# highfem/tqdne

Measured on AMD Instinct MI355X. Metric: waveforms/sec (train step + 18-step EDM sample), 3ch x 4096, higher is better.
Workload: dtype f32 (contractions on MFMA with fp32 accumulate: bf16x3, and fp16 + block-scaled-fp6 corrections on the 128/256-channel forward convs; sampler state f64)

## Files before the change

### tqdne_amd/csrc/backward.hip

```cpp
#include <cstdlib>
#include "common.hpp"
#include "../../include/tqdne_hip.h"

using namespace tq;

namespace {

typedef short s16x4 __attribute__((ext_vector_type(4)));

__device__ __forceinline__ f32x4 wg_mma(const bf16x8& ah, const bf16x8& al, const bf16x8& bh, const bf16x8& bl, f32x4 c) {
#if defined(TQ_WG_ABL_HIHI)
    return mfma_bf16(ah, bh, c);
#elif defined(TQ_WG_ABL_HALF)
    c = mfma_bf16(ah, bl, c);
    return mfma_bf16(ah, bh, c);
#else
    return mfma_x3(ah, al, bh, bl, c);
#endif
}

__device__ __forceinline__ uint2 lds_tr_read(const unsigned char* p) {
    s16x4 v = __builtin_amdgcn_ds_read_tr16_b64_v4i16((__attribute__((address_space(3))) s16x4*)(p));
    union { s16x4 s; uint2 u; } c;
    c.s = v;
// ... 187 lines not shown
                if (p.flags & TQ_CONV_SILU) {
#pragma unroll
                    for (int j = 0; j < 4; ++j) v[j] = silu_f(v[j]);
                }
                if (p.flags & TQ_CONV_DROPOUT) {
                    const uint32_t e0 = (uint32_t)pos * (uint32_t)Cin + (uint32_t)(cb + 4 * m);
                    const DropKey dkey = drop_key(p.drop_seed, p.drop_site, (uint32_t)b);
#pragma unroll
                    for (int j = 0; j < 4; ++j)
                        v[j] = (drop_hash(dkey, e0 + j) >= p.drop_thresh) ? v[j] * p.drop_scale : 0.f;
                }
            }
            bf16x4 h, l;
#pragma unroll
            for (int j = 0; j < 4; ++j) { __bf16 hh, ll; split_bf16(v[j], hh, ll); h[j] = hh; l[j] = ll; }
            const int off = i * WG_X_STRIDE + (W8 ? ((m * 8) ^ wg_x_swz128(i)) : (NCI == 1 ? ((m * 8) ^ wg_x_swz(i)) : (NCI == 4 ? ((m * 8) ^ wg_x_swz256(i)) : m * 8)));
            *reinterpret_cast<bf16x4*>(x_hi + off) = h;
            *reinterpret_cast<bf16x4*>(x_lo + off) = l;
        }
    };

    f32x4 acc[2][2 * NCI][KT];
#pragma unroll
    for (int i = 0; i < 2; ++i)
#pragma unroll
        for (int j = 0; j < 2 * NCI; ++j)
#pragma unroll
            for (int k = 0; k < KT; ++k) acc[i][j][k] = f32x4{0.f, 0.f, 0.f, 0.f};

    const int g = lane >> 4, q = (lane >> 2) & 3, pp = lane & 3;

    auto x_off = [&](int xrow, int nb) -> int __attribute__((always_inline)) {
        const int colx = ((wci * 2 + nb) * 16 + 4 * pp) * 2;
        return xrow * WG_X_STRIDE + (W8 ? (colx ^ wg_x_swz128(xrow)) : (NCI == 1 ? (colx ^ wg_x_swz(xrow)) : (NCI == 4 ? (colx ^ wg_x_swz256(xrow)) : colx)));
    };
    auto a_frags = [&](int r0, Frag (&ah)[2], Frag (&al)[2]) __attribute__((always_inline)) {
#pragma unroll
        for (int mb = 0; mb < 2; ++mb) {
            const int col = (wave * 32 + mb * 16 + 4 * pp) * 2;
            const int off = r0 * WG_DY_STRIDE + (col ^ wg_dy_swz<NCI>(r0));
            const int off4 = off + 4 * WG_DY_STRIDE;
            ah[mb].h[0] = lds_tr_read(dy_hi + off);
            ah[mb].h[1] = lds_tr_read(dy_hi + off4);
            al[mb].h[0] = lds_tr_read(dy_lo + off);
            al[mb].h[1] = lds_tr_read(dy_lo + off4);
        }
    };
#if !defined(TQ_WG_OLD_COMPUTE)
    struct XWin { uint2 h[3], l[3]; };
    auto x_window = [&](int r0, int nb, XWin& w) __attribute__((always_inline)) {
#pragma unroll
        for (int j = 0; j < 3; ++j) {
            const int off = x_off(r0 + 4 * j, nb);
            w.h[j] = lds_tr_read(x_hi + off);
            w.l[j] = lds_tr_read(x_lo + off);
        }
    };
    auto tap_frag = [&](const uint2 (&r)[3], const uint32_t (&al5)[5], int k, Frag& f) __attribute__((always_inline)) {
        const uint32_t d[6] = {r[0].x, r[0].y, r[1].x, r[1].y, r[2].x, r[2].y};
        if ((k & 1) == 0) f.u = make_uint4(d[k / 2], d[k / 2 + 1], d[k / 2 + 2], d[k / 2 + 3]);
        else f.u = make_uint4(al5[k / 2], al5[k / 2 + 1], al5[k / 2 + 2], al5[k / 2 + 3]);
    };
    auto compute = [&]() __attribute__((always_inline)) {
        if constexpr (STRIDE == 1 && KT > 1) {
            constexpr int NB = 2 * NCI, NG = (WG_TT / 32) * NB;
            XWin win[2];
            Frag ah[2], al[2];
            x_window(8 * g + q, 0, win[0]);
#pragma unroll
            for (int gi = 0; gi < NG; ++gi) {
                const int ks = gi / NB, nb = gi % NB;
                const int r0 = ks * 32 + 8 * g + q;
                if (nb == 0) a_frags(r0, ah, al);
                if (gi + 1 < NG) x_window(((gi + 1) / NB) * 32 + 8 * g + q, (gi + 1) % NB, win[(gi + 1) & 1]);
                __builtin_amdgcn_sched_barrier(0);
                const XWin& w = win[gi & 1];
                const uint32_t dh[6] = {w.h[0].x, w.h[0].y, w.h[1].x, w.h[1].y, w.h[2].x, w.h[2].y};
                const uint32_t dl[6] = {w.l[0].x, w.l[0].y, w.l[1].x, w.l[1].y, w.l[2].x, w.l[2].y};
                uint32_t oh[5], ol[5];
#pragma unroll
                for (int j = 0; j < (KT == 5 ? 5 : 4); ++j) {
                    oh[j] = __builtin_amdgcn_alignbit(dh[j + 1], dh[j], 16);
                    ol[j] = __builtin_amdgcn_alignbit(dl[j + 1], dl[j], 16);
                }
                if (KT != 5) { oh[4] = 0; ol[4] = 0; }
#pragma unroll
                for (int k = 0; k < KT; ++k) {
                    Frag bh, bl;
                    tap_frag(w.h, oh, k, bh);
                    tap_frag(w.l, ol, k, bl);
#pragma unroll
                    for (int mb = 0; mb < 2; ++mb)
                        acc[mb][nb][k] = wg_mma(ah[mb].v, al[mb].v, bh.v, bl.v, acc[mb][nb][k]);
                }
                __builtin_amdgcn_sched_barrier(0);
            }
            return;
        }
#else
    auto compute = [&]() __attribute__((always_inline)) {
#endif
#pragma unroll (NCI == 2 && KT == 5 ? 1 : 2)
        for (int ks = 0; ks < WG_TT / 32; ++ks) {
            const int r0 = ks * 32 + 8 * g + q;
            Frag ah[2], al[2];
            a_frags(r0, ah, al);
#pragma unroll
            for (int k = 0; k < KT; ++k) {
                const int xrow = (STRIDE == 1) ? (r0 + k) : ((k & 1) * (WG_TT + 1) + r0 + (k >> 1));
#pragma unroll
                for (int nb = 0; nb < 2 * NCI; ++nb) {
                    const int off = x_off(xrow, nb);
                    const int off4 = x_off(xrow + 4, nb);
                    Frag bh, bl;
                    bh.h[0] = lds_tr_read(x_hi + off);
                    bh.h[1] = lds_tr_read(x_hi + off4);
                    bl.h[0] = lds_tr_read(x_lo + off);
                    bl.h[1] = lds_tr_read(x_lo + off4);
#pragma unroll
                    for (int mb = 0; mb < 2; ++mb)
                        acc[mb][nb][k] = wg_mma(ah[mb].v, al[mb].v, bh.v, bl.v, acc[mb][nb][k]);
                }
            }
        }
    };

    constexpr bool PREFETCH = !(NCI == 2 && KT == 5);
    if (PREFETCH && u_begin < u_end) load_unit(u_begin);
    for (int u = u_begin; u < u_end; ++u) {
#ifdef TQ_WG_ABL_NOLOAD
        if (!PREFETCH && u == u_begin) load_unit(u);
#else
        if (!PREFETCH) load_unit(u);
#endif
        __syncthreads();
#ifdef TQ_WG_ABL_NOSTAGE
        if (u == u_begin)
#endif
        write_unit(u);
        __syncthreads();
#ifndef TQ_WG_ABL_NOLOAD
        if (PREFETCH && u + 1 < u_end) load_unit(u + 1);
#endif
#ifndef TQ_WG_ABL_NOMMA
        if (wave_active) compute();
#endif
    }

    if (do_cs) {
        __syncthreads();
        cs_flush();
    }
    if (!wave_active) return;
#pragma unroll
    for (int k = 0; k < KT; ++k)
#pragma unroll
        for (int mb = 0; mb < 2; ++mb)
#pragma unroll
            for (int nb = 0; nb < 2 * NCI; ++nb)
#pragma unroll
                for (int r = 0; r < 4; ++r) {
                    const int co = co0 + wave * 32 + mb * 16 + 4 * (lane >> 4) + r;
                    const int ci = cb + (wci * 2 + nb) * 16 + (lane & 15);
                    p.slab[(((size_t)sp * KT + k) * p.C_out + co) * Cin + ci] = acc[mb][nb][k][r];
                }
}

template <int KT>
__global__ __launch_bounds__(256) void wgrad_reduce_kernel(const float* __restrict__ slab, float* __restrict__ dw, int nsplit, size_t n) {
    __shared__ __attribute__((aligned(16))) float red[16][KT][68];
    const int x = threadIdx.x, y = threadIdx.y;
    const size_t i0 = (size_t)blockIdx.x * 64;
    const size_t i = i0 + 4 * x;
    float4 acc[KT];
#pragma unroll
    for (int k = 0; k < KT; ++k) acc[k] = make_float4(0.f, 0.f, 0.f, 0.f);
    if (i < n) {
        const float* base = slab + i;
        int sidx = y;
        for (; sidx + 16 < nsplit; sidx += 32) {
            float4 v0[KT], v1[KT];
#pragma unroll
            for (int k = 0; k < KT; ++k) {
                v0[k] = *reinterpret_cast<const float4*>(base + ((size_t)sidx * KT + k) * n);
                v1[k] = *reinterpret_cast<const float4*>(base + ((size_t)(sidx + 16) * KT + k) * n);
            }
#pragma unroll
            for (int k = 0; k < KT; ++k) {
                acc[k].x += v0[k].x + v1[k].x; acc[k].y += v0[k].y + v1[k].y;
                acc[k].z += v0[k].z + v1[k].z; acc[k].w += v0[k].w + v1[k].w;
            }
        }
        if (sidx < nsplit) {
#pragma unroll
            for (int k = 0; k < KT; ++k) {
                const float4 v = *reinterpret_cast<const float4*>(base + ((size_t)sidx * KT + k) * n);
                acc[k].x += v.x; acc[k].y += v.y; acc[k].z += v.z; acc[k].w += v.w;
            }
        }
    }
#pragma unroll
    for (int k = 0; k < KT; ++k) *reinterpret_cast<float4*>(&red[y][k][4 * x]) = acc[k];
    __syncthreads();
    const int tid = y * 16 + x;
    const size_t nleft = n - i0 < 64 ? n - i0 : 64;
    for (int o = tid; o < (int)nleft * KT; o += 256) {
        const int il = o / KT, k = o - il * KT;
        float t = 0.f;
#pragma unroll
        for (int q = 0; q < 16; ++q) t += red[q][k][il];
        dw[i0 * KT + o] = t;
    }
}

int wgrad_nci(const TqConvDesc* d) {
    static const int forced = [] { const char* e = getenv("TQDNE_WGRAD_NCI"); return e ? atoi(e) : 0; }();
    if (forced == 1) return 1;
    if (d->ktaps != 1 && forced != 2) return 1;
    if (d->ktaps == 1 && d->stride == 1 && !d->upsample && forced != 2 && d->C_in0 % 128 == 0 && d->C_in1 % 128 == 0) return 4;
    return (d->C_in0 % 64 == 0 && d->C_in1 % 64 == 0) ? 2 : 1;
}

bool wgrad_w8(const TqConvDesc* d) {
    static const int sw = [] { const char* e = getenv("TQDNE_WGRAD_W8"); return e ? atoi(e) : 1; }();
    if (!sw || d->ktaps == 1) return false;
    return d->C_in0 % 64 == 0 && d->C_in1 % 64 == 0 && d->C_out % 128 == 0;
}

bool wgrad_h64(const TqConvDesc* d) {
    static const int sw = [] { const char* e = getenv("TQDNE_WGRAD_H64"); return e ? atoi(e) : 1; }();
    if (!sw || d->ktaps == 1 || d->stride != 1 || d->upsample) return false;
    return d->C_in0 % 64 == 0 && d->C_in1 % 64 == 0 && d->C_out == 64;
}

template <int KT, int STRIDE, int UPS>
size_t wgrad_lds(int nci, bool w8) {
    constexpr int XR = (STRIDE == 1) ? (WG_TT + KT - 1) : (2 * WG_TT + 1);
    const int ncx = w8 ? 2 : nci;
    return 2 * WG_TT * ((nci == 1 || nci == 4) ? WG_DY_STRIDE1 : WG_DY_STRIDE2) + 2 * XR * 64 * ncx + 128 * sizeof(float);
}

template <int KT, int STRIDE, int UPS, int NCI, bool W8, bool H64 = false>
int wgrad_slots_of() {
    static const int slots = [] {
        const size_t sh = wgrad_lds<KT, STRIDE, UPS>(NCI, W8);
        int per_cu = 0, dev = 0, cus = 0;
        if (hipGetDevice(&dev) != hipSuccess || hipDeviceGetAttribute(&cus, hipDeviceAttributeMultiprocessorCount, dev) != hipSuccess ||
            hipOccupancyMaxActiveBlocksPerMultiprocessor(&per_cu, wgrad_kernel<KT, STRIDE, UPS, NCI, W8, H64>, (W8 && !H64) ? 512 : 256, sh) != hipSuccess ||
            per_cu < 1 || cus < 1) {
            (void)hipGetLastError();
            return (W8 && !H64) ? 256 : 512;
        }
        return per_cu * cus;
    }();
    return slots;
}

template <int KT, int STRIDE, int UPS>
int wgrad_slots_k(int nci, bool w8, bool h64 = false) {
    if constexpr (KT != 1 && STRIDE == 1 && UPS == 0) {
        if (h64) return wgrad_slots_of<KT, STRIDE, UPS, 1, true, true>();
    }
    if (w8) return wgrad_slots_of<KT, STRIDE, UPS, 1, true>();
    if constexpr (KT == 1 && STRIDE == 1 && UPS == 0) {
        if (nci == 4) return wgrad_slots_of<KT, STRIDE, UPS, 4, false>();
    }
    return nci == 2 ? wgrad_slots_of<KT, STRIDE, UPS, 2, false>() : wgrad_slots_of<KT, STRIDE, UPS, 1, false>();
}

int wgrad_slots(const TqConvDesc* d, int nci, bool w8, bool h64) {
    if (d->stride == 2) return wgrad_slots_k<3, 2, 0>(nci, w8);
    if (d->upsample) return d->ktaps == 5 ? wgrad_slots_k<5, 1, 1>(nci, w8) : wgrad_slots_k<3, 1, 1>(nci, w8);
    if (d->ktaps == 5) return wgrad_slots_k<5, 1, 0>(nci, w8, h64);
    if (d->ktaps == 3) return wgrad_slots_k<3, 1, 0>(nci, w8, h64);
    return wgrad_slots_k<1, 1, 0>(nci, false);
}

void wgrad_plan(const TqConvDesc* d, bool wide, int& n_cotiles, int& n_cichunks, int& n_ttiles, int& nsplit, int& ups) {
    const int nci = wgrad_nci(d);
    const bool h64 = wide && wgrad_h64(d);
    const bool w8 = wide && (h64 || wgrad_w8(d));
    n_cotiles = h64 ? 1 : (d->C_out + 127) / 128;
    n_cichunks = (d->C_in0 + d->C_in1) / (32 * (w8 ? 2 : nci));
    n_ttiles = (d->T_out + WG_TT - 1) / WG_TT;
    const int U = d->B * n_ttiles;
    const int ntiles = n_cotiles * n_cichunks;
    static const int forced = [] { const char* e = getenv("TQDNE_WGRAD_SLOTS"); return e ? atoi(e) : 0; }();
    const int slots = forced > 0 ? forced : wgrad_slots(d, nci, w8, h64);
    int want = slots / ntiles;
    if (want < 1) want = 1;
    if (want > U) want = U;
    ups = (U + want - 1) / want;
    nsplit = (U + ups - 1) / ups;
}

template <int KT, int STRIDE, int UPS>
int launch_wgrad(const WgArgs& a, int nci, bool w8, bool h64, hipStream_t stream) {
    const size_t sh = wgrad_lds<KT, STRIDE, UPS>(nci, w8 || h64);
    const unsigned grid = (unsigned)(a.n_cotiles * a.n_cichunks * a.nsplit);
    if (h64) {
        if constexpr (KT != 1 && STRIDE == 1 && UPS == 0) {
            hipLaunchKernelGGL((wgrad_kernel<KT, STRIDE, UPS, 1, true, true>), dim3(grid), dim3(256), sh, stream, a);
        } else {
            return TQ_ERR_SHAPE;
        }
    } else if (w8) {
        static const bool raised = [] {
            return hipFuncSetAttribute(reinterpret_cast<const void*>(wgrad_kernel<KT, STRIDE, UPS, 1, true>),
                                       hipFuncAttributeMaxDynamicSharedMemorySize, 160 * 1024) == hipSuccess;
        }();
        (void)raised;
        hipLaunchKernelGGL((wgrad_kernel<KT, STRIDE, UPS, 1, true>), dim3(grid), dim3(512), sh, stream, a);
    } else if (nci == 4) {
        if constexpr (KT == 1 && STRIDE == 1 && UPS == 0) {
            static const bool raised4 = [] {
                return hipFuncSetAttribute(reinterpret_cast<const void*>(wgrad_kernel<1, 1, 0, 4, false>),
                                           hipFuncAttributeMaxDynamicSharedMemorySize, 80 * 1024) == hipSuccess;
            }();
            (void)raised4;
            hipLaunchKernelGGL((wgrad_kernel<1, 1, 0, 4, false>), dim3(grid), dim3(256), sh, stream, a);
        } else {
            return TQ_ERR_SHAPE;
        }
    } else if (nci == 2) {
        hipLaunchKernelGGL((wgrad_kernel<KT, STRIDE, UPS, 2, false>), dim3(grid), dim3(256), sh, stream, a);
    } else {
        hipLaunchKernelGGL((wgrad_kernel<KT, STRIDE, UPS, 1, false>), dim3(grid), dim3(256), sh, stream, a);
    }
    TQ_CHECK_LAUNCH();
    return 0;
}
}

extern "C" size_t tq_conv1d_bwd_weight_workspace(const TqConvDesc* d) {
    if (!d) return 0;
    int a, b, c, nsplit, nsplit4, ups;
    wgrad_plan(d, true, a, b, c, nsplit, ups);
    wgrad_plan(d, false, a, b, c, nsplit4, ups);
    return (size_t)(nsplit > nsplit4 ? nsplit : nsplit4) * d->ktaps * d->C_out * (d->C_in0 + d->C_in1) * sizeof(float);
}

extern "C" int tq_conv1d_bwd_weight(const TqConvDesc* d, const float* dy, const float* x0, const float* x1,
                                    const float* gscale, const float* gshift, float* dw, void* workspace, size_t ws_bytes,
                                    hipStream_t stream) {
    return tq_conv1d_bwd_weight_colsum(d, dy, x0, x1, gscale, gshift, dw, workspace, ws_bytes, nullptr, 0, nullptr, nullptr, stream);
}

extern "C" int tq_conv1d_bwd_weight_colsum(const TqConvDesc* d, const float* dy, const float* x0, const float* x1,
                                           const float* gscale, const float* gshift, float* dw, void* workspace, size_t ws_bytes,
                                           float* colsum_bc, int bc_stride, float* colsum_c, float* colsum_c2,
                                           hipStream_t stream) {
    if (!d || !dy || !x0 || !dw || !workspace) return TQ_ERR_ARG;
    if (colsum_c2 && !colsum_c) return TQ_ERR_ARG;
    if (d->C_in0 <= 0 || d->C_in0 % 32 || d->C_in1 < 0 || d->C_in1 % 32 || d->C_out <= 0 || d->C_out % 32) return TQ_ERR_SHAPE;
    if (d->C_in1 > 0 && !x1) return TQ_ERR_ARG;
    if ((d->flags & TQ_CONV_GN) && (!gscale || !gshift)) return TQ_ERR_ARG;
    if (ws_bytes < tq_conv1d_bwd_weight_workspace(d)) return TQ_ERR_ARG;
    WgArgs a;
    a.dy = dy; a.x0 = x0; a.x1 = x1; a.gscale = gscale; a.gshift = gshift; a.slab = reinterpret_cast<float*>(workspace);
    a.B = d->B; a.T_in = d->T_in; a.T_out = d->T_out; a.C0 = d->C_in0; a.C1 = d->C_in1; a.C_out = d->C_out;
    a.flags = d->flags;
    a.cs_bc = colsum_bc; a.cs_stride = bc_stride; a.cs_c = colsum_c; a.cs_c2 = colsum_c2;
    const bool wide = !(colsum_bc || colsum_c);
    wgrad_plan(d, wide, a.n_cotiles, a.n_cichunks, a.n_ttiles, a.nsplit, a.units_per_split);
    static const bool plain_order = [] { const char* e = getenv("TQDNE_WGRAD_XCD"); return e && atoi(e) == 0; }();
    if (plain_order) a.flags |= TQ_WGRAD_PLAIN_ORDER;
    a.drop_site = d->dropout_site; a.drop_seed = d->dropout_seed;
    float pdrop = d->dropout_p;
    if (!(d->flags & TQ_CONV_DROPOUT) || pdrop <= 0.f) { a.flags &= ~TQ_CONV_DROPOUT; pdrop = 0.f; }
    a.drop_thresh = (uint32_t)((double)pdrop * 4294967296.0);
    a.drop_scale = 1.0f / (1.0f - pdrop);
    int rc;
    const int nci = wgrad_nci(d);
    const bool h64 = wide && wgrad_h64(d);
    const bool w8 = wide && !h64 && wgrad_w8(d);
    if (d->stride == 2) {
        if (d->ktaps != 3) return TQ_ERR_SHAPE;
        rc = launch_wgrad<3, 2, 0>(a, nci, w8, false, stream);
    } else if (d->upsample) {
        if (d->ktaps == 5) rc = launch_wgrad<5, 1, 1>(a, nci, w8, false, stream);
        else if (d->ktaps == 3) rc = launch_wgrad<3, 1, 1>(a, nci, w8, false, stream);
        else return TQ_ERR_SHAPE;
    } else {
        if (d->ktaps == 5) rc = launch_wgrad<5, 1, 0>(a, nci, w8, h64, stream);
        else if (d->ktaps == 3) rc = launch_wgrad<3, 1, 0>(a, nci, w8, h64, stream);
        else if (d->ktaps == 1) rc = launch_wgrad<1, 1, 0>(a, nci, false, false, stream);
        else return TQ_ERR_SHAPE;
    }
    if (rc) return rc;
    const size_t n = (size_t)d->C_out * (d->C_in0 + d->C_in1);
    const dim3 rgrid((unsigned)((n + 63) / 64)), rblock(16, 16);
    if (d->ktaps == 5) hipLaunchKernelGGL(wgrad_reduce_kernel<5>, rgrid, rblock, 0, stream, a.slab, dw, a.nsplit, n);
    else if (d->ktaps == 3) hipLaunchKernelGGL(wgrad_reduce_kernel<3>, rgrid, rblock, 0, stream, a.slab, dw, a.nsplit, n);
    else hipLaunchKernelGGL(wgrad_reduce_kernel<1>, rgrid, rblock, 0, stream, a.slab, dw, a.nsplit, n);
    TQ_CHECK_LAUNCH();
    return 0;
}

namespace {
__global__ __launch_bounds__(256) void gn_bwd_finalize_kernel(const float* __restrict__ gst, const float* __restrict__ mr,
                                                              const float* __restrict__ gamma, int C, int T, int nslots,
                                                              float* __restrict__ cA, float* __restrict__ cB,
                                                              float* __restrict__ cC, float* __restrict__ dgamma,
                                                              float* __restrict__ dbeta) {
    extern __shared__ double sh[];
    const int b = blockIdx.x;
    const int Cb = C / (int)gridDim.y;
    const int c0 = (int)blockIdx.y * Cb;
    int nsub = Cb <= 128 ? (int)blockDim.x / Cb : 1;
    if (nsub > nslots) nsub = nslots;
    double* cs = sh;
    double* gp = sh + 2 * Cb * nsub;
    for (int idx = threadIdx.x; idx < Cb * nsub; idx += blockDim.x) {
        const int c = idx % Cb, sub = idx / Cb;
        const float* pp = gst + ((size_t)b * nslots * C + c0 + c) * 2;
        double s1 = 0.0, s2 = 0.0;
        int s = sub;
        for (; s + 3 * nsub < nslots; s += 4 * nsub) {
            const float2 v0 = *reinterpret_cast<const float2*>(pp + (size_t)s * C * 2);
            const float2 v1 = *reinterpret_cast<const float2*>(pp + (size_t)(s + nsub) * C * 2);
            const float2 v2 = *reinterpret_cast<const float2*>(pp + (size_t)(s + 2 * nsub) * C * 2);
            const float2 v3 = *reinterpret_cast<const float2*>(pp + (size_t)(s + 3 * nsub) * C * 2);
            s1 += ((double)v0.x + (double)v1.x) + ((double)v2.x + (double)v3.x);
            s2 += ((double)v0.y + (double)v1.y) + ((double)v2.y + (double)v3.y);
        }
        for (; s < nslots; s += nsub) {
            const float2 v = *reinterpret_cast<const float2*>(pp + (size_t)s * C * 2);
            s1 += (double)v.x; s2 += (double)v.y;
        }
        cs[2 * idx] = s1; cs[2 * idx + 1] = s2;
    }
    __syncthreads();
    if (nsub > 1) {
        double t1 = 0.0, t2 = 0.0;
        const int c = threadIdx.x;
        if (c < Cb)
            for (int sub = 0; sub < nsub; ++sub) { t1 += cs[2 * (sub * Cb + c)]; t2 += cs[2 * (sub * Cb + c) + 1]; }
        __syncthreads();
        if (c < Cb) { cs[2 * c] = t1; cs[2 * c + 1] = t2; }
        __syncthreads();
    }
    const int G = C / GN_GROUPS;
    const int ngrp = Cb / G, g0 = c0 / G;
    if ((int)threadIdx.x < ngrp) {
        const int gl = threadIdx.x, g = g0 + gl;
        const double mean = (double)mr[((size_t)b * GN_GROUPS + g) * 2], rstd = (double)mr[((size_t)b * GN_GROUPS + g) * 2 + 1];
        double p1 = 0.0, p2 = 0.0;
        for (int j = 0; j < G; ++j) {
            const int cl = gl * G + j;
            const double gm = (double)gamma[c0 + cl];
            p1 += gm * cs[2 * cl];
            p2 += gm * (cs[2 * cl + 1] - mean * cs[2 * cl]);
        }
        p2 *= rstd;
        const double n = (double)G * (double)T;
        gp[2 * gl] = -rstd * rstd * p2 / n;
        gp[2 * gl + 1] = rstd * rstd * p2 * mean / n - rstd * p1 / n;
    }
    __syncthreads();
    for (int cl = threadIdx.x; cl < Cb; cl += blockDim.x) {
        const int c = c0 + cl;
        const int g = c / G, gl = g - g0;
        const float mean = mr[((size_t)b * GN_GROUPS + g) * 2], rstd = mr[((size_t)b * GN_GROUPS + g) * 2 + 1];
        cA[(size_t)b * C + c] = rstd * gamma[c];
        cB[(size_t)b * C + c] = (float)gp[2 * gl];
        cC[(size_t)b * C + c] = (float)gp[2 * gl + 1];
        atomicAdd(dgamma + c, (float)((double)rstd * (cs[2 * cl + 1] - (double)mean * cs[2 * cl])));
        atomicAdd(dbeta + c, (float)cs[2 * cl]);
    }
}

__global__ void gn_bwd_apply_kernel(const float* __restrict__ g, const float* __restrict__ x, const float* __restrict__ r,
                                    const float* __restrict__ cA, const float* __restrict__ cB, const float* __restrict__ cC,
                                    float* __restrict__ dx, int T, int Cs, int Ctot, int coff, int accum, size_t n4) {
    const int c4n = Cs >> 2;
    for (size_t i = (size_t)blockIdx.x * blockDim.x + threadIdx.x; i < n4; i += (size_t)gridDim.x * blockDim.x) {
        const int c4 = (int)(i % c4n);
        const size_t bt = i / c4n;
        const int b = (int)(bt / T);
        const size_t ko = (size_t)b * Ctot + coff + 4 * c4;
        const float4 a = *reinterpret_cast<const float4*>(cA + ko);
        const float4 bb = *reinterpret_cast<const float4*>(cB + ko);
        const float4 cc = *reinterpret_cast<const float4*>(cC + ko);
        const float4 gv = reinterpret_cast<const float4*>(g)[i];
        const float4 xv = reinterpret_cast<const float4*>(x)[i];
        float4 o = make_float4(a.x * gv.x + bb.x * xv.x + cc.x, a.y * gv.y + bb.y * xv.y + cc.y,
                               a.z * gv.z + bb.z * xv.z + cc.z, a.w * gv.w + bb.w * xv.w + cc.w);
        if (r) { const float4 rv = reinterpret_cast<const float4*>(r)[i]; o.x += rv.x; o.y += rv.y; o.z += rv.z; o.w += rv.w; }
        if (accum) { const float4 ov = reinterpret_cast<const float4*>(dx)[i]; o.x += ov.x; o.y += ov.y; o.z += ov.z; o.w += ov.w; }
        reinterpret_cast<float4*>(dx)[i] = o;
    }
}

constexpr int AMAX_WAYS = TQ_AMAX_WAYS;
constexpr int AMAX_STRIDE = TQ_AMAX_STRIDE;

template <int NT>
__device__ __forceinline__ void colsum_finish(float* red, const float4& a, float mx, bool active, int c4n, int nrow, int c4, int tr, int C,
                                              int b, float sc, float* __restrict__ out_bc, int bc_stride, float* __restrict__ out_c,
                                              float* __restrict__ out_c2, unsigned* __restrict__ amax_out) {
    if (active) *reinterpret_cast<float4*>(red + (tr * c4n + c4) * 4) = a;
    unsigned* wmax = reinterpret_cast<unsigned*>(red + (size_t)nrow * c4n * 4);
    if (amax_out) {
        unsigned m = __float_as_uint(mx);
#pragma unroll
        for (int o = 32; o > 0; o >>= 1) m = max(m, (unsigned)__shfl_xor((int)m, o));
        if ((threadIdx.x & 63) == 0) wmax[threadIdx.x >> 6] = m;
    }
    __syncthreads();
    if (amax_out && threadIdx.x == 0) {
        unsigned m = wmax[0];
#pragma unroll
        for (int w = 1; w < NT / 64; ++w) m = max(m, wmax[w]);
        if (m != 0u) atomicMax(amax_out + (blockIdx.x % AMAX_WAYS) * AMAX_STRIDE, m);
    }
    for (int c = threadIdx.x; c < C; c += NT) {
        float s = 0.f;
        for (int r2 = 0; r2 < nrow; ++r2) s += red[(r2 * c4n + (c >> 2)) * 4 + (c & 3)];
        s *= sc;
        if (out_bc) atomicAdd(out_bc + (size_t)b * bc_stride + c, s);
        if (out_c) atomicAdd(out_c + c, s);
        if (out_c2) atomicAdd(out_c2 + c, s);
    }
}
__device__ __forceinline__ float amax4(float m, const float4& v) {
    const float t = fmaxf(fmaxf(fabsf(v.x), fabsf(v.y)), fmaxf(fabsf(v.z), fabsf(v.w)));
    const bool bad = (v.x != v.x) | (v.y != v.y) | (v.z != v.z) | (v.w != v.w);
    return bad ? __builtin_inff() : fmaxf(m, t);
}

template <int NT>
__global__ __launch_bounds__(NT) void colsum_kernel(const float* __restrict__ dy, int T, int C, float* __restrict__ out_bc,
                                                     int bc_stride, float* __restrict__ out_c, float* __restrict__ out_c2,
                                                     const float* __restrict__ bscale, unsigned* __restrict__ amax_out, int rpw) {
    extern __shared__ float red[];
    const int nsl = (T + rpw - 1) / rpw;
    const int slot = blockIdx.x % nsl, b = blockIdx.x / nsl;
    const int c4n = C >> 2;
    const int nrow = NT / c4n > 0 ? NT / c4n : 1;
    const int c4 = threadIdx.x % c4n, tr = threadIdx.x / c4n;
    float4 a = make_float4(0.f, 0.f, 0.f, 0.f);
    float mx = 0.f;
    const bool active = tr < nrow && threadIdx.x < nrow * c4n;
    if (active) {
        const int nvalid = min(rpw, T - slot * rpw);
        const float* src = dy + ((size_t)b * T + (size_t)slot * rpw) * C + 4 * c4;
        int tl = tr;
        for (; tl + 7 * nrow < nvalid; tl += 8 * nrow) {
            float4 v[8];
#pragma unroll
            for (int q = 0; q < 8; ++q) v[q] = *reinterpret_cast<const float4*>(src + (size_t)(tl + q * nrow) * C);
#pragma unroll
            for (int q = 0; q < 8; ++q) { a.x += v[q].x; a.y += v[q].y; a.z += v[q].z; a.w += v[q].w; }
            if (amax_out) {
#pragma unroll
                for (int q = 0; q < 8; ++q) mx = amax4(mx, v[q]);
            }
        }
        for (; tl < nvalid; tl += nrow) {
            const float4 v = *reinterpret_cast<const float4*>(src + (size_t)tl * C);
            a.x += v.x; a.y += v.y; a.z += v.z; a.w += v.w;
            if (amax_out) mx = amax4(mx, v);
        }
    }
    colsum_finish<NT>(red, a, mx, active, c4n, nrow, c4, tr, C, b, bscale ? bscale[b] : 1.0f, out_bc, bc_stride, out_c, out_c2, amax_out);
}

template <int NT>
__global__ __launch_bounds__(NT) void gn_bwd_apply_cs_kernel(const float* __restrict__ g, const float* __restrict__ x,
                                                              const float* __restrict__ r, const float* __restrict__ cA,
                                                              const float* __restrict__ cB, const float* __restrict__ cC,
                                                              float* __restrict__ dx, int T, int Cs, int Ctot, int coff, int accum,
                                                              float* __restrict__ out_bc, int bc_stride, float* __restrict__ out_c,
                                                              float* __restrict__ out_c2, unsigned* __restrict__ amax_out, int rpw) {
    extern __shared__ float red[];
    const int nsl = (T + rpw - 1) / rpw;
    const int slot = blockIdx.x % nsl, b = blockIdx.x / nsl;
    const int c4n = Cs >> 2;
    const int nrow = NT / c4n > 0 ? NT / c4n : 1;
    const int c4 = threadIdx.x % c4n, tr = threadIdx.x / c4n;
    float4 a = make_float4(0.f, 0.f, 0.f, 0.f);
    float mx = 0.f;
    const bool active = tr < nrow && threadIdx.x < nrow * c4n;
    if (active) {
        const int nvalid = min(rpw, T - slot * rpw);
        const size_t ko = (size_t)b * Ctot + coff + 4 * c4;
        const float4 ka = *reinterpret_cast<const float4*>(cA + ko);
        const float4 kb = *reinterpret_cast<const float4*>(cB + ko);
        const float4 kc = *reinterpret_cast<const float4*>(cC + ko);
        const size_t base = ((size_t)b * T + (size_t)slot * rpw) * Cs + 4 * c4;
        auto one = [&](const float4& gv, const float4& xv, const float4& rv, const float4& ov) -> float4 __attribute__((always_inline)) {
            float4 o = make_float4(ka.x * gv.x + kb.x * xv.x + kc.x, ka.y * gv.y + kb.y * xv.y + kc.y,
                                   ka.z * gv.z + kb.z * xv.z + kc.z, ka.w * gv.w + kb.w * xv.w + kc.w);
            o.x += rv.x; o.y += rv.y; o.z += rv.z; o.w += rv.w;
            o.x += ov.x; o.y += ov.y; o.z += ov.z; o.w += ov.w;
            return o;
        };
        const float4 z4 = make_float4(0.f, 0.f, 0.f, 0.f);
        int tl = tr;
        for (; tl + 3 * nrow < nvalid; tl += 4 * nrow) {
            float4 gv[4], xv[4], rv[4], ov[4];
#pragma unroll
            for (int q = 0; q < 4; ++q) {
                const size_t o = base + (size_t)(tl + q * nrow) * Cs;
                gv[q] = *reinterpret_cast<const float4*>(g + o);
                xv[q] = *reinterpret_cast<const float4*>(x + o);
                rv[q] = r ? *reinterpret_cast<const float4*>(r + o) : z4;
                ov[q] = accum ? *reinterpret_cast<const float4*>(dx + o) : z4;
            }
#pragma unroll
            for (int q = 0; q < 4; ++q) {
                const float4 o4 = one(gv[q], xv[q], rv[q], ov[q]);
                *reinterpret_cast<float4*>(dx + base + (size_t)(tl + q * nrow) * Cs) = o4;
                a.x += o4.x; a.y += o4.y; a.z += o4.z; a.w += o4.w;
                mx = amax4(mx, o4);
            }
        }
        for (; tl < nvalid; tl += nrow) {
            const size_t o = base + (size_t)tl * Cs;
            const float4 o4 = one(*reinterpret_cast<const float4*>(g + o), *reinterpret_cast<const float4*>(x + o),
                                  r ? *reinterpret_cast<const float4*>(r + o) : z4, accum ? *reinterpret_cast<const float4*>(dx + o) : z4);
            *reinterpret_cast<float4*>(dx + o) = o4;
            a.x += o4.x; a.y += o4.y; a.z += o4.z; a.w += o4.w;
            mx = amax4(mx, o4);
        }
    }
    colsum_finish<NT>(red, a, mx, active, c4n, nrow, c4, tr, Cs, b, 1.0f, out_bc, bc_stride, out_c, out_c2, amax_out);
}

__global__ void zero_stuff_kernel(const float* __restrict__ dy, float* __restrict__ out, int T_out, int T_in, int C, size_t n4) {
    const int c4n = C >> 2;
    for (size_t i = (size_t)blockIdx.x * blockDim.x + threadIdx.x; i < n4; i += (size_t)gridDim.x * blockDim.x) {
        const int c4 = (int)(i % c4n);
        const size_t bu = i / c4n;
        const int u = (int)(bu % T_in);
        const size_t b = bu / T_in;
        float4 v = make_float4(0.f, 0.f, 0.f, 0.f);
        if (!(u & 1) && (u >> 1) < T_out) v = reinterpret_cast<const float4*>(dy)[(b * T_out + (u >> 1)) * c4n + c4];
        reinterpret_cast<float4*>(out)[i] = v;
    }
}

__global__ void pair_sum_kernel(const float* __restrict__ dup, float* __restrict__ dx, int T, int C, int accum, size_t n4) {
    const int c4n = C >> 2;
    for (size_t i = (size_t)blockIdx.x * blockDim.x + threadIdx.x; i < n4; i += (size_t)gridDim.x * blockDim.x) {
        const int c4 = (int)(i % c4n);
        const size_t bt = i / c4n;
        const int t = (int)(bt % T);
        const size_t b = bt / T;
        const float4 a = reinterpret_cast<const float4*>(dup)[(b * 2 * T + 2 * t) * c4n + c4];
        const float4 c = reinterpret_cast<const float4*>(dup)[(b * 2 * T + 2 * t + 1) * c4n + c4];
        float4 o = make_float4(a.x + c.x, a.y + c.y, a.z + c.z, a.w + c.w);
        if (accum) { const float4 ov = reinterpret_cast<const float4*>(dx)[i]; o.x += ov.x; o.y += ov.y; o.z += ov.z; o.w += ov.w; }
        reinterpret_cast<float4*>(dx)[i] = o;
    }
}

inline unsigned ew_grid4(size_t n4) {
    size_t g = (n4 + 255) / 256;
    return (unsigned)(g > 4096 ? 4096 : (g ? g : 1));
}
}

extern "C" int tq_gn_bwd_finalize(const float* gstats, const float* mean_rstd, const float* gamma, int B, int C, int T,
                                  float* coef_a, float* coef_b, float* coef_c, float* dgamma, float* dbeta,
                                  hipStream_t stream) {
    if (!gstats || !mean_rstd || !gamma || !coef_a || !coef_b || !coef_c || !dgamma || !dbeta) return TQ_ERR_ARG;
    if (B <= 0 || T <= 0 || C <= 0 || C % GN_GROUPS) return TQ_ERR_SHAPE;
    const int nslots = (T + STAT_SLOT - 1) / STAT_SLOT;
    static const int forced = [] { const char* e = getenv("TQDNE_GNBWD_PARTS"); return e ? atoi(e) : 0; }();
    const int NP = (forced == 1 || forced == 2 || forced == 4 || forced == 8) ? forced : 4;
    const int Cb = C / NP;
    int nsub = Cb <= 128 ? 256 / Cb : 1;
    if (nsub > nslots) nsub = nslots;
    const size_t sh = (size_t)(2 * Cb * nsub + 2 * GN_GROUPS) * sizeof(double);
    hipLaunchKernelGGL(gn_bwd_finalize_kernel, dim3(B, NP), dim3(256), sh, stream, gstats, mean_rstd, gamma, C, T, nslots, coef_a,
                       coef_b, coef_c, dgamma, dbeta);
    TQ_CHECK_LAUNCH();
    return 0;
}

extern "C" int tq_gn_bwd_apply(const float* g, const float* x, const float* r, const float* coef_a, const float* coef_b,
                               const float* coef_c, float* dx, int B, int T, int C_src, int C_total, int c_offset, int accumulate,
                               hipStream_t stream) {
    if (!g || !x || !coef_a || !coef_b || !coef_c || !dx) return TQ_ERR_ARG;
    if (B <= 0 || T <= 0 || C_src <= 0 || C_src % 4 || c_offset % 4 || c_offset + C_src > C_total) return TQ_ERR_SHAPE;
    const size_t n4 = (size_t)B * T * (C_src / 4);
    hipLaunchKernelGGL(gn_bwd_apply_kernel, dim3(ew_grid4(n4)), dim3(256), 0, stream, g, x, r, coef_a, coef_b, coef_c, dx, T,
                       C_src, C_total, c_offset, accumulate, n4);
    TQ_CHECK_LAUNCH();
    return 0;
}

struct CsTiling { int nt, rows; };
static CsTiling colsum_tiling(int B, int T) {
    static const int f_nt = [] { const char* e = getenv("TQDNE_COLSUM_THREADS"); return e ? atoi(e) : 0; }();
    static const int f_rows = [] { const char* e = getenv("TQDNE_COLSUM_ROWS"); return e ? atoi(e) : 0; }();
    static const int f_wgs = [] { const char* e = getenv("TQDNE_COLSUM_WGS"); return e ? atoi(e) : 0; }();
    CsTiling t;
    t.nt = f_nt == 1024 ? 1024 : 256;
    const size_t min_wgs = f_wgs > 0 ? (size_t)f_wgs : 256;
    int rpw = STAT_SLOT;
    while (rpw < 4096 && (size_t)B * ((T + 2 * rpw - 1) / (2 * rpw)) >= min_wgs) rpw <<= 1;
    t.rows = f_rows > 0 ? f_rows : rpw;
    return t;
}

extern "C" int tq_colsum(const float* dy, int B, int T, int C, float* out_bc, int bc_stride, float* out_c, float* out_c2,
                         const float* bscale, uint32_t* amax_out, hipStream_t stream) {
    if (!dy || (!out_bc && !out_c && !out_c2 && !amax_out)) return TQ_ERR_ARG;
    if (B <= 0 || T <= 0 || C < 4 || C % 4 || C > 1024) return TQ_ERR_SHAPE;
    const CsTiling tl = colsum_tiling(B, T);
    const int nsl = (T + tl.rows - 1) / tl.rows;
    const int c4n = C / 4;
    const int nrow = tl.nt / c4n > 0 ? tl.nt / c4n : 1;
    const size_t sh = (size_t)nrow * c4n * 4 * sizeof(float) + (tl.nt / 64) * sizeof(unsigned);
    if (tl.nt == 1024)
        hipLaunchKernelGGL(colsum_kernel<1024>, dim3(B * nsl), dim3(1024), sh, stream, dy, T, C, out_bc, bc_stride, out_c, out_c2, bscale, amax_out, tl.rows);
    else
        hipLaunchKernelGGL(colsum_kernel<256>, dim3(B * nsl), dim3(256), sh, stream, dy, T, C, out_bc, bc_stride, out_c, out_c2, bscale, amax_out, tl.rows);
    TQ_CHECK_LAUNCH();
    return 0;
}

extern "C" int tq_gn_bwd_apply_colsum(const float* g, const float* x, const float* r, const float* coef_a, const float* coef_b,
                                      const float* coef_c, float* dx, int B, int T, int C_src, int C_total, int c_offset, int accumulate,
                                      float* colsum_bc, int bc_stride, float* colsum_c, float* colsum_c2, uint32_t* amax_out,
                                      hipStream_t stream) {
    if (!g || !x || !coef_a || !coef_b || !coef_c || !dx) return TQ_ERR_ARG;
    if (colsum_c2 && !colsum_c) return TQ_ERR_ARG;
    if (B <= 0 || T <= 0 || C_src <= 0 || C_src % 4 || C_src > 1024 || c_offset % 4 || c_offset + C_src > C_total) return TQ_ERR_SHAPE;
    if (!colsum_bc && !colsum_c && !amax_out)
        return tq_gn_bwd_apply(g, x, r, coef_a, coef_b, coef_c, dx, B, T, C_src, C_total, c_offset, accumulate, stream);
    const CsTiling tl = colsum_tiling(B, T);
    const int nsl = (T + tl.rows - 1) / tl.rows;
    const int c4n = C_src / 4;
    const int nrow = tl.nt / c4n > 0 ? tl.nt / c4n : 1;
    const size_t sh = (size_t)nrow * c4n * 4 * sizeof(float) + (tl.nt / 64) * sizeof(unsigned);
    if (tl.nt == 1024)
        hipLaunchKernelGGL(gn_bwd_apply_cs_kernel<1024>, dim3(B * nsl), dim3(1024), sh, stream, g, x, r, coef_a, coef_b, coef_c, dx, T, C_src,
                           C_total, c_offset, accumulate, colsum_bc, bc_stride, colsum_c, colsum_c2, amax_out, tl.rows);
    else
        hipLaunchKernelGGL(gn_bwd_apply_cs_kernel<256>, dim3(B * nsl), dim3(256), sh, stream, g, x, r, coef_a, coef_b, coef_c, dx, T, C_src,
                           C_total, c_offset, accumulate, colsum_bc, bc_stride, colsum_c, colsum_c2, amax_out, tl.rows);
    TQ_CHECK_LAUNCH();
    return 0;
}

extern "C" int tq_zero_stuff(const float* dy, float* out, int B, int T_out, int T_in, int C, hipStream_t stream) {
    if (!dy || !out || B <= 0 || T_out <= 0 || T_in <= 0 || C % 4) return TQ_ERR_ARG;
    const size_t n4 = (size_t)B * T_in * (C / 4);
    hipLaunchKernelGGL(zero_stuff_kernel, dim3(ew_grid4(n4)), dim3(256), 0, stream, dy, out, T_out, T_in, C, n4);
    TQ_CHECK_LAUNCH();
    return 0;
}

extern "C" int tq_pair_sum(const float* d_up, float* dx, int B, int T, int C, int accumulate, hipStream_t stream) {
    if (!d_up || !dx || B <= 0 || T <= 0 || C % 4) return TQ_ERR_ARG;
    const size_t n4 = (size_t)B * T * (C / 4);
    hipLaunchKernelGGL(pair_sum_kernel, dim3(ew_grid4(n4)), dim3(256), 0, stream, d_up, dx, T, C, accumulate, n4);
    TQ_CHECK_LAUNCH();
    return 0;
}

namespace {
__global__ __launch_bounds__(256) void poly_wgrad_fold_kernel(const float* __restrict__ dw2, float* __restrict__ dw, int n) {
    const int i = blockIdx.x * 256 + threadIdx.x;
    if (i >= n) return;
    const float* a = dw2 + (size_t)i * 3;
    const float* b = dw2 + ((size_t)n + i) * 3;
    const float a0 = a[0], a1 = a[1], a2 = a[2], b0 = b[0], b1 = b[1], b2 = b[2];
    float* o = dw + (size_t)i * 5;
    o[0] = a0 + b0; o[1] = a0 + b1; o[2] = a1 + b1; o[3] = a1 + b2; o[4] = a2 + b2;
}
}

extern "C" int tq_upsample_poly_wgrad_fold(const float* dw2, float* dw, int C_out, int C_in, hipStream_t stream) {
    if (!dw2 || !dw || C_out <= 0 || C_in <= 0) return TQ_ERR_ARG;
    const int n = C_out * C_in;
    hipLaunchKernelGGL(poly_wgrad_fold_kernel, dim3((unsigned)((n + 255) / 256)), dim3(256), 0, stream, dw2, dw, n);
    TQ_CHECK_LAUNCH();
    return 0;
}

namespace {
template <int KT, int CI>
__global__ __launch_bounds__(256) void stem_wgrad_stream_kernel(const float* __restrict__ dy, const float* __restrict__ x,
                                                                const float* __restrict__ in_scale, float* __restrict__ dw,
                                                                float* __restrict__ part, int C_in, int T, int C_out, int nslots,
                                                                int nunits, int upw) {
    extern __shared__ float shm[];
    constexpr int PAD = KT / 2, TW = STAT_SLOT + KT - 1, BLK = 16;
    float* xs = shm;
    float* red = xs + CI * TW;
    const int nseg = 256 / C_out, L = STAT_SLOT / nseg;
    const int co = threadIdx.x % C_out, seg = threadIdx.x / C_out;
    float acc[CI][KT];
#pragma unroll
    for (int ci = 0; ci < CI; ++ci)
#pragma unroll
        for (int k = 0; k < KT; ++k) acc[ci][k] = 0.f;
    const int u0 = blockIdx.x * upw, u1 = min(nunits, u0 + upw);
    for (int u = u0; u < u1; ++u) {
        const int slot = u % nslots, b = u / nslots;
        const int t0 = slot * STAT_SLOT;
        const float sc = in_scale ? in_scale[b] : 1.0f;
        __syncthreads();
        for (int i = threadIdx.x; i < C_in * TW; i += 256) {
            const int c = i / TW, j = i % TW;
            const int t = t0 - PAD + j;
            xs[c * TW + j] = (t >= 0 && t < T) ? x[((size_t)b * C_in + c) * T + t] * sc : 0.f;
        }
        __syncthreads();
        const int tb = t0 + seg * L;
        for (int tl = 0; tl < L; tl += BLK) {
            float d[BLK];
#pragma unroll
            for (int j = 0; j < BLK; ++j) {
                const int tj = tb + tl + j;
                const int tc = tj < T ? tj : T - 1;
                d[j] = dy[((size_t)b * T + tc) * C_out + co] * (tj < T ? 1.f : 0.f);
            }
#pragma unroll
            for (int ci = 0; ci < CI; ++ci) {
                if (ci < C_in) {
                    float xw[BLK + KT - 1];
#pragma unroll
                    for (int j = 0; j < BLK + KT - 1; ++j) xw[j] = xs[ci * TW + seg * L + tl + j];
#pragma unroll
                    for (int j = 0; j < BLK; ++j)
// ... 509 lines not shown
```

Before: 352.8.

## Restructure GroupNorm backward finalize to one block per group, dropping atomics

The GroupNorm backward finalize kernel now launches one 1024-thread block per group. Each block loops over batch chunks, instead of using a (batch, channel-part) grid whose blocks atomically add into dgamma and dbeta. Per-channel dgamma and dbeta are accumulated in shared memory across the batch and written once with plain adds, which removes atomic contention and makes the reduction order deterministic. The cost is a small grid of GN_GROUPS blocks that walk the batch serially, which may leave much of the GPU idle for large B. Separately, ablation macros are added to skip the wgrad slab write and the reduce launch; they are inactive by default.

Measured after the change: 351.7 (median of 2 runs). Within noise of the previous version (-0.3%).

```diff
diff --git a/tqdne_amd/csrc/backward.hip b/tqdne_amd/csrc/backward.hip
--- a/tqdne_amd/csrc/backward.hip
+++ b/tqdne_amd/csrc/backward.hip
@@ -363,6 +363,9 @@
         cs_flush();
     }
     if (!wave_active) return;
+#ifdef TQ_WG_ABL_NOSLAB
+    if (p.nsplit >= 0) return;
+#endif
 #pragma unroll
     for (int k = 0; k < KT; ++k)
 #pragma unroll
@@ -599,6 +602,9 @@
         else return TQ_ERR_SHAPE;
     }
     if (rc) return rc;
+#if defined(TQ_WG_ABL_NOSLAB) || defined(TQ_WG_ABL_NOREDUCE)
+    return 0;
+#endif
     const size_t n = (size_t)d->C_out * (d->C_in0 + d->C_in1);
     const dim3 rgrid((unsigned)((n + 63) / 64)), rblock(16, 16);
     if (d->ktaps == 5) hipLaunchKernelGGL(wgrad_reduce_kernel<5>, rgrid, rblock, 0, stream, a.slab, dw, a.nsplit, n);
@@ -609,75 +615,95 @@
 }
 
 namespace {
-__global__ __launch_bounds__(256) void gn_bwd_finalize_kernel(const float* __restrict__ gst, const float* __restrict__ mr,
-                                                              const float* __restrict__ gamma, int C, int T, int nslots,
-                                                              float* __restrict__ cA, float* __restrict__ cB,
-                                                              float* __restrict__ cC, float* __restrict__ dgamma,
-                                                              float* __restrict__ dbeta) {
+constexpr int GNB_NT = 1024;
+constexpr int GNB_ITEMS = 2048;
+
+inline int gnb_nsub(int C, int nslots) {
+    const int Cb = C / 4;
+    const int nsub = Cb <= 128 ? 256 / Cb : 1;
+    return nsub < nslots ? nsub : nslots;
+}
+
+__global__ __launch_bounds__(GNB_NT) void gn_bwd_finalize_kernel(const float* __restrict__ gst, const float* __restrict__ mr,
+                                                                 const float* __restrict__ gamma, int B, int C, int T, int nslots,
+                                                                 int nsub, int bb, float* __restrict__ cA, float* __restrict__ cB,
+                                                                 float* __restrict__ cC, float* __restrict__ dgamma,
+                                                                 float* __restrict__ dbeta) {
     extern __shared__ double sh[];
-    const int b = blockIdx.x;
-    const int Cb = C / (int)gridDim.y;
-    const int c0 = (int)blockIdx.y * Cb;
-    int nsub = Cb <= 128 ? (int)blockDim.x / Cb : 1;
-    if (nsub > nslots) nsub = nslots;
+    const int G = C / GN_GROUPS;
+    const int g = blockIdx.x, c0 = g * G;
     double* cs = sh;
-    double* gp = sh + 2 * Cb * nsub;
-    for (int idx = threadIdx.x; idx < Cb * nsub; idx += blockDim.x) {
-        const int c = idx % Cb, sub = idx / Cb;
-        const float* pp = gst + ((size_t)b * nslots * C + c0 + c) * 2;
-        double s1 = 0.0, s2 = 0.0;
-        int s = sub;
-        for (; s + 3 * nsub < nslots; s += 4 * nsub) {
-            const float2 v0 = *reinterpret_cast<const float2*>(pp + (size_t)s * C * 2);
-            const float2 v1 = *reinterpret_cast<const float2*>(pp + (size_t)(s + nsub) * C * 2);
-            const float2 v2 = *reinterpret_cast<const float2*>(pp + (size_t)(s + 2 * nsub) * C * 2);
-            const float2 v3 = *reinterpret_cast<const float2*>(pp + (size_t)(s + 3 * nsub) * C * 2);
-            s1 += ((double)v0.x + (double)v1.x) + ((double)v2.x + (double)v3.x);
-            s2 += ((double)v0.y + (double)v1.y) + ((double)v2.y + (double)v3.y);
-        }
-        for (; s < nslots; s += nsub) {
-            const float2 v = *reinterpret_cast<const float2*>(pp + (size_t)s * C * 2);
-            s1 += (double)v.x; s2 += (double)v.y;
-        }
-        cs[2 * idx] = s1; cs[2 * idx + 1] = s2;
-    }
-    __syncthreads();
-    if (nsub > 1) {
-        double t1 = 0.0, t2 = 0.0;
-        const int c = threadIdx.x;
-        if (c < Cb)
-            for (int sub = 0; sub < nsub; ++sub) { t1 += cs[2 * (sub * Cb + c)]; t2 += cs[2 * (sub * Cb + c) + 1]; }
-        __syncthreads();
-        if (c < Cb) { cs[2 * c] = t1; cs[2 * c + 1] = t2; }
-        __syncthreads();
-    }
-    const int G = C / GN_GROUPS;
-    const int ngrp = Cb / G, g0 = c0 / G;
-    if ((int)threadIdx.x < ngrp) {
-        const int gl = threadIdx.x, g = g0 + gl;
-        const double mean = (double)mr[((size_t)b * GN_GROUPS + g) * 2], rstd = (double)mr[((size_t)b * GN_GROUPS + g) * 2 + 1];
-        double p1 = 0.0, p2 = 0.0;
-        for (int j = 0; j < G; ++j) {
-            const int cl = gl * G + j;
-            const double gm = (double)gamma[c0 + cl];
-            p1 += gm * cs[2 * cl];
-            p2 += gm * (cs[2 * cl + 1] - mean * cs[2 * cl]);
-        }
-        p2 *= rstd;
-        const double n = (double)G * (double)T;
-        gp[2 * gl] = -rstd * rstd * p2 / n;
-        gp[2 * gl + 1] = rstd * rstd * p2 * mean / n - rstd * p1 / n;
-    }
-    __syncthreads();
-    for (int cl = threadIdx.x; cl < Cb; cl += blockDim.x) {
-        const int c = c0 + cl;
-        const int g = c / G, gl = g - g0;
-        const float mean = mr[((size_t)b * GN_GROUPS + g) * 2], rstd = mr[((size_t)b * GN_GROUPS + g) * 2 + 1];
-        cA[(size_t)b * C + c] = rstd * gamma[c];
-        cB[(size_t)b * C + c] = (float)gp[2 * gl];
-        cC[(size_t)b * C + c] = (float)gp[2 * gl + 1];
-        atomicAdd(dgamma + c, (float)((double)rstd * (cs[2 * cl + 1] - (double)mean * cs[2 * cl])));
-        atomicAdd(dbeta + c, (float)cs[2 * cl]);
+    double* gp = sh + 2 * bb * G * nsub;
+    double* acc = gp + 2 * bb;
+    for (int i = threadIdx.x; i < 2 * G; i += GNB_NT) acc[i] = 0.0;
+    const double n = (double)G * (double)T;
+    for (int b0 = 0; b0 < B; b0 += bb) {
+        const int nb = min(bb, B - b0);
+        for (int idx = threadIdx.x; idx < nb * G * nsub; idx += GNB_NT) {
+            const int sub = idx % nsub, c = (idx / nsub) % G, bl = idx / (nsub * G);
+            const float* pp = gst + ((size_t)(b0 + bl) * nslots * C + c0 + c) * 2;
+            double s1 = 0.0, s2 = 0.0;
+            int s = sub;
+            for (; s + 3 * nsub < nslots; s += 4 * nsub) {
+                const float2 v0 = *reinterpret_cast<const float2*>(pp + (size_t)s * C * 2);
+                const float2 v1 = *reinterpret_cast<const float2*>(pp + (size_t)(s + nsub) * C * 2);
+                const float2 v2 = *reinterpret_cast<const float2*>(pp + (size_t)(s + 2 * nsub) * C * 2);
+                const float2 v3 = *reinterpret_cast<const float2*>(pp + (size_t)(s + 3 * nsub) * C * 2);
+                s1 += ((double)v0.x + (double)v1.x) + ((double)v2.x + (double)v3.x);
+                s2 += ((double)v0.y + (double)v1.y) + ((double)v2.y + (double)v3.y);
+            }
+            for (; s < nslots; s += nsub) {
+                const float2 v = *reinterpret_cast<const float2*>(pp + (size_t)s * C * 2);
+                s1 += (double)v.x; s2 += (double)v.y;
+            }
+            cs[2 * idx] = s1; cs[2 * idx + 1] = s2;
+        }
+        __syncthreads();
+        if (nsub > 1) {
+            for (int bc = threadIdx.x; bc < nb * G; bc += GNB_NT) {
+                double t1 = 0.0, t2 = 0.0;
+                for (int sub = 0; sub < nsub; ++sub) { t1 += cs[2 * (bc * nsub + sub)]; t2 += cs[2 * (bc * nsub + sub) + 1]; }
+                cs[2 * bc * nsub] = t1; cs[2 * bc * nsub + 1] = t2;
+            }
+            __syncthreads();
+        }
+        for (int bl = threadIdx.x; bl < nb; bl += GNB_NT) {
+            const int b = b0 + bl;
+            const double mean = (double)mr[((size_t)b * GN_GROUPS + g) * 2], rstd = (double)mr[((size_t)b * GN_GROUPS + g) * 2 + 1];
+            double p1 = 0.0, p2 = 0.0;
+            for (int j = 0; j < G; ++j) {
+                const double* t = cs + 2 * ((bl * G + j) * nsub);
+                const double gm = (double)gamma[c0 + j];
+                p1 += gm * t[0];
+                p2 += gm * (t[1] - mean * t[0]);
+            }
+            p2 *= rstd;
+            gp[2 * bl] = -rstd * rstd * p2 / n;
+            gp[2 * bl + 1] = rstd * rstd * p2 * mean / n - rstd * p1 / n;
+        }
+        __syncthreads();
+        for (int bc = threadIdx.x; bc < nb * G; bc += GNB_NT) {
+            const int bl = bc / G, cl = bc - bl * G, b = b0 + bl, c = c0 + cl;
+            const float mean = mr[((size_t)b * GN_GROUPS + g) * 2], rstd = mr[((size_t)b * GN_GROUPS + g) * 2 + 1];
+            cA[(size_t)b * C + c] = rstd * gamma[c];
+            cB[(size_t)b * C + c] = (float)gp[2 * bl];
+            cC[(size_t)b * C + c] = (float)gp[2 * bl + 1];
+            double* t = cs + 2 * bc * nsub;
+            const double s1 = t[0];
+            t[0] = (double)rstd * (t[1] - (double)mean * s1);
+            t[1] = s1;
+        }
+        __syncthreads();
+        for (int cl = threadIdx.x; cl < G; cl += GNB_NT) {
+            double ag = acc[2 * cl], ab = acc[2 * cl + 1];
+            for (int bl = 0; bl < nb; ++bl) { ag += cs[2 * (bl * G + cl) * nsub]; ab += cs[2 * (bl * G + cl) * nsub + 1]; }
+            acc[2 * cl] = ag; acc[2 * cl + 1] = ab;
+        }
+        __syncthreads();
+    }
+    for (int cl = threadIdx.x; cl < G; cl += GNB_NT) {
+        dgamma[c0 + cl] += (float)acc[2 * cl];
+        dbeta[c0 + cl] += (float)acc[2 * cl + 1];
     }
 }
 
@@ -879,14 +905,15 @@
     if (!gstats || !mean_rstd || !gamma || !coef_a || !coef_b || !coef_c || !dgamma || !dbeta) return TQ_ERR_ARG;
     if (B <= 0 || T <= 0 || C <= 0 || C % GN_GROUPS) return TQ_ERR_SHAPE;
     const int nslots = (T + STAT_SLOT - 1) / STAT_SLOT;
-    static const int forced = [] { const char* e = getenv("TQDNE_GNBWD_PARTS"); return e ? atoi(e) : 0; }();
-    const int NP = (forced == 1 || forced == 2 || forced == 4 || forced == 8) ? forced : 4;
-    const int Cb = C / NP;
-    int nsub = Cb <= 128 ? 256 / Cb : 1;
-    if (nsub > nslots) nsub = nslots;
-    const size_t sh = (size_t)(2 * Cb * nsub + 2 * GN_GROUPS) * sizeof(double);
-    hipLaunchKernelGGL(gn_bwd_finalize_kernel, dim3(B, NP), dim3(256), sh, stream, gstats, mean_rstd, gamma, C, T, nslots, coef_a,
-                       coef_b, coef_c, dgamma, dbeta);
+    const int G = C / GN_GROUPS;
+    const int nsub = gnb_nsub(C, nslots);
+    int bb = GNB_ITEMS / (G * nsub);
+    if (bb < 1) bb = 1;
+    if (bb > B) bb = B;
+    const size_t sh = (size_t)(2 * bb * G * nsub + 2 * bb + 2 * G) * sizeof(double);
+    if (sh > 64 * 1024) return TQ_ERR_SHAPE;
+    hipLaunchKernelGGL(gn_bwd_finalize_kernel, dim3(GN_GROUPS), dim3(GNB_NT), sh, stream, gstats, mean_rstd, gamma, B, C, T, nslots, nsub, bb,
+                       coef_a, coef_b, coef_c, dgamma, dbeta);
     TQ_CHECK_LAUNCH();
     return 0;
 }
```
